# amisr/volumetricinterp

Measured on AMD Instinct MI355X. Metric: fit+eval timesteps/sec, higher is better.
Workload: dtype f64

## Files before the change

### volumetricinterp_amd/csrc/vi_brent.hip

```cpp
#include "vi_solver.h"
#include "vi_jacobi_device.h"
#include "vi_jacobi_v2_device.h"
#include "vi_gemm_device.h"
#include "vi_exp10.h"

#include <cstdlib>
#include <cstring>


#ifdef VI_STAMPS
__device__ unsigned long long g_brent_stamps[16];
__device__ unsigned long long g_brent_hist[64][2];
#define BR_STAMP(k)                                                                   \
    do {                                                                              \
        const unsigned long long t_ = __builtin_readcyclecounter();                   \
        if (threadIdx.x == 0) atomicAdd(&g_brent_stamps[k], t_ - stamp_t);            \
        stamp_t = __builtin_readcyclecounter();                                       \
    } while (0)
#else
#define BR_STAMP(k)
#endif

namespace {

struct BrentState {
    double xpre, xcur, xblk, fpre, fcur, fblk, spre, scur;
    double last_x;
    int it, funcalls, done, status;
    int nreq, rebased, rebase_now;
};

struct RebaseRule {
    double sched[4];
    int nsched;
    int again_after;
    double again_within;
    int again_on;
    double jump_width, jump_frac;
};

__host__ inline int rule_from_host(const double* h, RebaseRule& rr)
{
    rr.nsched = (int)h[0];
    if (rr.nsched < 0 || rr.nsched > 4) return -1;
    for (int i = 0; i < 4; ++i) rr.sched[i] = h[1 + i];
    rr.again_after = (int)h[5];
    rr.again_within = h[6];
    rr.again_on = (int)h[7];
    rr.jump_width = h[8];
    rr.jump_frac = h[9];
    return 0;
}

__host__ __device__ __forceinline__ void rebase_decide(BrentState& s, const RebaseRule& rr)
{
    const double x = s.xcur;
    bool rb = false;
    if (s.last_x == s.last_x) {
        const double d = fabs(x - s.last_x);
        if (s.rebased < rr.nsched)
            rb = d < rr.sched[s.rebased];
        else
            rb = rr.again_on && s.rebased == rr.nsched && s.nreq >= rr.again_after && d < rr.again_within;
    }
// ... 1 lines not shown
    s.rebase_now = rb ? 1 : 0;
    s.last_x = x;
    s.nreq += 1;
}

__host__ __device__ __forceinline__ bool brent_top(BrentState& s, double xtol, double rtol, double jump_width, double jump_fmin)
{
#pragma clang fp contract(off)
    if (s.fpre != 0.0 && s.fcur != 0.0 && (signbit(s.fpre) != signbit(s.fcur))) {
        s.xblk = s.xpre;
        s.fblk = s.fpre;
        s.spre = s.scur = s.xcur - s.xpre;
    }
    if (fabs(s.fblk) < fabs(s.fcur)) {
        const double xp = s.xcur, xc = s.xblk, xb = s.xcur;
        const double fp = s.fcur, fc = s.fblk, fb = s.fcur;
        s.xpre = xp; s.xcur = xc; s.xblk = xb;
        s.fpre = fp; s.fcur = fc; s.fblk = fb;
    }
    const double delta = (xtol + rtol * fabs(s.xcur)) / 2;
    const double sbis = (s.xblk - s.xcur) / 2;
    if (s.fcur == 0.0 || fabs(sbis) < delta) return true;
    if (jump_width > 0.0 && fabs(s.xblk - s.xcur) <= jump_width && fabs(s.fcur) > jump_fmin) return true;
    if (fabs(s.spre) > delta && fabs(s.fcur) < fabs(s.fpre)) {
        double stry;
        if (s.xpre == s.xblk) {
            stry = -s.fcur * (s.xcur - s.xpre) / (s.fcur - s.fpre);
        } else {
            const double dpre = (s.fpre - s.fcur) / (s.xpre - s.xcur);
            const double dblk = (s.fblk - s.fcur) / (s.xblk - s.xcur);
            stry = -s.fcur * (s.fblk * dblk - s.fpre * dpre) / (dblk * dpre * (s.fblk - s.fpre));
        }
        const double a = fabs(s.spre), b = 3 * fabs(sbis) - delta;
        if (2 * fabs(stry) < (b < a ? b : a)) {
            s.spre = s.scur;
            s.scur = stry;
        } else {
            s.spre = sbis;
            s.scur = sbis;
        }
    } else {
        s.spre = sbis;
        s.scur = sbis;
    }
    s.xpre = s.xcur;
    s.fpre = s.fcur;
    if (fabs(s.scur) > delta)
        s.xcur += s.scur;
    else
        s.xcur += (sbis > 0 ? delta : -delta);
    return false;
}

template <int IT>
__device__ __noinline__ void jacobi_system_call(unsigned char* lds_raw, int N, const double* Xs, double sc, const double* ys,
                                                double rcond, double abs_floor, double* Cs, double2* logp, int max_sweeps,
                                                int* sweeps_s, int* nround_s, unsigned long long* round_acc)
{
    if constexpr (IT == 0)
        jacobi_system_v2(lds_raw, N, Xs, sc, ys, rcond, abs_floor, Cs, nullptr, logp, max_sweeps, sweeps_s, nullptr, 0, nround_s,
                         round_acc);
    else
        jacobi_system<IT>(lds_raw, N, Xs, sc, ys, rcond, abs_floor, Cs, nullptr, logp, max_sweeps, sweeps_s, nullptr, 0, nround_s,
                          round_acc);
}

__device__ __noinline__ void rebase_call(unsigned char* lds_raw, int N, const double2* logp, int64_t nround, double* Vs,
                                         double* VwS, double* VnS, const double* AWAr, const double* Rm, double* D1s, double* D2s,
                                         const double* yr, double* yts
#ifdef VI_STAMPS
                                         , unsigned long long& stamp_t
#endif
                                         )
{
    const int tid = threadIdx.x, NT = blockDim.x, nw = NT >> 6, lane = tid & 63, wave = tid >> 6;
    const int NN = N * N;
    for (int col0 = wave * 4; col0 < N; col0 += nw * 4) jacobi_vector_strip<4>(N, logp, nround, col0, lane, VwS);
    __syncthreads();
    BR_STAMP(6);
    double* ldsg = reinterpret_cast<double*>(lds_raw);
    wg_gemm<false>(N, Vs, VwS, VnS, ldsg);
    for (int e = tid; e < NN; e += NT) Vs[e] = VnS[e];
    __syncthreads();
    wg_gemm<false>(N, AWAr, VnS, VwS, ldsg);
    wg_gemm<true>(N, VnS, VwS, D1s, ldsg);
    wg_gemm<false>(N, Rm, VnS, VwS, ldsg);
    wg_gemm<true>(N, VnS, VwS, D2s, ldsg);
    for (int k = wave; k < N; k += nw) {
        double acc = 0.0;
        for (int r = lane; r < N; r += 64) acc = fma(VnS[(int64_t)k * N + r], yr[r], acc);
        for (int o2 = 32; o2 > 0; o2 >>= 1) acc += __shfl_down(acc, o2);
        if (lane == 0) yts[k] = acc;
    }
    __syncthreads();
}

template <int IT>
__global__ __launch_bounds__(IT <= 1 ? 768 : 512) void k_brent_warm(
    int N, int64_t P, int ntask, double* D1, double* D2, double* yt, double* V, const double* __restrict__ AWA,
    const double* __restrict__ Rm, const double* __restrict__ ysrc, RebaseRule rr, double* __restrict__ VwW, double* __restrict__ VnW,
    const double* __restrict__ At, const double* __restrict__ W, const double* __restrict__ b,
    const int* __restrict__ t_rec, const int* __restrict__ t_slot, const double* __restrict__ t_xa,
    const double* __restrict__ t_xb, const double* __restrict__ t_fa, const double* __restrict__ t_fb,
    const double* __restrict__ t_nu, double rcond, double abs_floor, int max_sweeps, double xtol, double rtol, int maxiter,
    int* __restrict__ queue, double* __restrict__ Xw, double2* __restrict__ logw, int64_t log_stride, double* __restrict__ cw,
    double* __restrict__ o_root, double* __restrict__ o_other, int* __restrict__ o_iters, int* __restrict__ o_funcalls,
    int* __restrict__ o_status, size_t lds_jacobi, int npart, unsigned long long* __restrict__ round_acc)
{
    extern __shared__ __align__(16) unsigned char lds_raw[];
    double* shC = reinterpret_cast<double*>(lds_raw + lds_jacobi);
    double* red = shC + ((N + 1) & ~1);
    double* part = red + 768;
    double* shd = part + npart;
    BrentState* st = reinterpret_cast<BrentState*>(shd + 16);
    int* shi = reinterpret_cast<int*>(st + 1);

    const int tid = threadIdx.x, NT = blockDim.x, nw = NT >> 6;
    const int NN = N * N;
    double* Xs = Xw + (int64_t)blockIdx.x * NN;
    double2* logp = logw + (int64_t)blockIdx.x * log_stride;
    double* cp = cw + (int64_t)blockIdx.x * N;
    double* VwS = VwW + (int64_t)blockIdx.x * NN;
    double* VnS = VnW + (int64_t)blockIdx.x * NN;
    const int nb = (int)((P + 255) / 256);

#ifdef VI_STAMPS
    unsigned long long stamp_t = __builtin_readcyclecounter();
    const unsigned long long wall0 = wall_clock64();
    if (threadIdx.x == 0) atomicMin(&g_brent_stamps[12], wall0);
#endif
    for (;;) {
        if (tid == 0) shi[0] = atomicAdd(queue, 1);
        __syncthreads();
        const int task = shi[0];
        if (task >= ntask) {
#ifdef VI_STAMPS
            if (threadIdx.x == 0) { const unsigned long long w1 = wall_clock64(); atomicAdd(&g_brent_stamps[11], w1 - wall0); atomicMax(&g_brent_stamps[13], w1); }
#endif
            break;
        }
        const int64_t slot = t_slot[task], rec = t_rec[task];
        const double nu = t_nu[task];
        double* D1s = D1 + slot * NN;
        double* D2s = D2 + slot * NN;
        double* Vs = V + slot * NN;
        const double* Wr = W + rec * P;
        const double* br = b + rec * P;
        if (tid == 0) {
            BrentState s;
            s.xpre = t_xa[task]; s.xcur = t_xb[task]; s.fpre = t_fa[task]; s.fcur = t_fb[task];
            s.xblk = s.fblk = s.spre = s.scur = 0.0;
            s.it = 1; s.funcalls = 0; s.status = 0;
            s.last_x = __builtin_nan("");
            s.nreq = 0; s.rebased = 0; s.rebase_now = 0;
            s.done = brent_top(s, xtol, rtol, rr.jump_width, rr.jump_frac * nu) ? 1 : 0;
            if (!s.done) rebase_decide(s, rr);
            *st = s;
        }
        __syncthreads();
        BR_STAMP(0);
        while (!st->done) {
            const double alpha = vi_exp10(st->xcur);
            double mx = 0.0;
            for (int e = tid; e < NN; e += NT) mx = fmax(mx, fabs(fma(alpha, D2s[e], D1s[e])));
            for (int o = 32; o > 0; o >>= 1) mx = fmax(mx, __shfl_xor(mx, o));
            if ((tid & 63) == 0) shd[tid >> 6] = mx;
            __syncthreads();
            mx = 0.0;
            for (int q = 0; q < nw; ++q) mx = fmax(mx, shd[q]);
            int ex = 0;
            double f = 1.0;
            if (mx > 0.0 && mx < 1.7e308) {
                (void)frexp(mx, &ex);
                f = ldexp(1.0, 1 - ex);
            }
            for (int e = tid; e < NN; e += NT) Xs[e] = fma(alpha, D2s[e], D1s[e]) * f;
            __syncthreads();
            BR_STAMP(1);
            if constexpr (IT == 3)
                jacobi_system<3>(lds_raw, N, Xs, 1.0 / f, yt + slot * N, rcond, abs_floor, cp, nullptr, logp, max_sweeps, shi + 1,
                                 nullptr, 0, shi + 2, round_acc);
            else
                jacobi_system_call<IT>(lds_raw, N, Xs, 1.0 / f, yt + slot * N, rcond, abs_floor, cp, logp, max_sweeps, shi + 1,
                                       shi + 2, round_acc);
            __syncthreads();
            BR_STAMP(2);
#ifdef VI_STAMPS
            if (tid == 0) { const int ii_ = st->it < 63 ? st->it : 63; atomicAdd(&g_brent_hist[ii_][0], (unsigned long long)shi[1]); atomicAdd(&g_brent_hist[ii_][1], 1ull); atomicAdd(&g_brent_stamps[8], (unsigned long long)shi[1]); atomicAdd(&g_brent_stamps[9], 1ull); atomicAdd(&g_brent_stamps[10], (unsigned long long)shi[2]); }
#endif
            for (int k = tid; k < N; k += NT) red[k] = cp[k];
            __syncthreads();
            for (int r = tid; r < N; r += NT) {
                double acc = 0.0;
                for (int k0 = 0; k0 < N; k0 += 16) {
                    double v[16];
#pragma unroll
                    for (int u = 0; u < 16; ++u) v[u] = (k0 + u < N) ? Vs[(int64_t)(k0 + u) * N + r] : 0.0;
#pragma unroll
                    for (int u = 0; u < 16; ++u)
                        if (k0 + u < N) acc = fma(v[u], red[k0 + u], acc);
                }
                shC[r] = acc;
            }
            __syncthreads();
            BR_STAMP(3);
            const int nbp = NT >> 8;
            for (int b0 = 0; b0 < nb; b0 += nbp) {
                const int sub = tid >> 8, t = tid & 255;
                const int blk = b0 + sub;
                double v = 0.0;
                if (sub < nbp && blk < nb) {
                    const int64_t p = (int64_t)blk * 256 + t;
                    if (p < P) {
                        double acc = 0.0;
#pragma unroll 8
                        for (int n = 0; n < N; ++n) acc = fma(At[(int64_t)n * P + p], shC[n], acc);
                        const double d = acc - br[p];
                        v = d * d * Wr[p];
                    }
                }
                if (sub < nbp) red[tid] = v;
                __syncthreads();
                for (int h = 128; h > 0; h >>= 1) {
                    if (sub < nbp && t < h) red[tid] += red[tid + h];
                    __syncthreads();
                }
                if (sub < nbp && t == 0 && blk < nb) part[blk] = red[tid];
                __syncthreads();
            }
            BR_STAMP(4);
            if (tid == 0) {
                double chi = 0.0;
                for (int j = 0; j < nb; ++j) chi += part[j];
                BrentState s = *st;
                if (shi[1] > max_sweeps) {
                    s.status = 2;
                    s.done = 1;
// ... 195 lines not shown
    h_out[3] = (double)s.funcalls;
    h_out[4] = (double)s.status;
    h_out[5] = (double)s.rebased;
    return VI_OK;
}

extern "C" int vi_brent_warm_f64(vi_ctx* c, int64_t ntask, int32_t N, int64_t P, double* d_D1, double* d_D2, double* d_yt,
                                 double* d_V, const double* d_AWA, const double* d_R, const double* d_y,
                                 const double* h_rebase ,
                                 const double* d_At, const double* d_W,
                                 const double* d_b, const int32_t* d_rec, const int32_t* d_slot, const double* d_xa,
                                 const double* d_xb, const double* d_fa, const double* d_fb, const double* d_nu, double rcond,
                                 double* d_root, double* d_other, int32_t* d_iters, int32_t* d_funcalls, int32_t* d_status)
{
    const double abs_floor = vi_floor_warm();
    const int max_sweeps = vi_max_sweeps();
    size_t ldsj_eff;
    VI_REQUIRE(c && d_D1 && d_D2 && d_yt && d_V && d_AWA && d_R && d_y && h_rebase && d_At && d_W && d_b && d_rec && d_slot && d_xa && d_xb && d_fa && d_fb && d_nu &&
                   d_root && d_other && d_iters && d_funcalls && d_status, "null argument");
    VI_REQUIRE(ntask >= 0 && N > 0 && P > 0, "bad size");
    if (ntask == 0) return VI_OK;
    if (!vi_jacobi_supported(N)) {
        vi_set_error("vi_brent_warm_f64: N=%d outside the in-LDS Jacobi range", N);
        return VI_ERR_UNSUPPORTED;
    }
    int npart;
    const size_t lds_all = brent_lds_bytes(N, P, &ldsj_eff, &npart);
    const size_t shm = lds_all - BRENT_STATIC_LDS;
    if (lds_all > VI_LDS_BYTES_PER_CU) {
        vi_set_error("vi_brent_warm_f64: %lld data points per record need %zu bytes of LDS (the chi^2 partial sums of a record "
                     "sit beside its rotated system); the host-driven iteration has no such limit", (long long)P, lds_all);
        return VI_ERR_UNSUPPORTED;
    }
    VI_HIP(hipSetDevice(c->device));
    int threads, it;
    brent_geometry(N, threads, it);
    const int64_t nwg = ntask < c->n_cu ? ntask : c->n_cu;
    const size_t logb = vi_jacobi_log_bytes(N, max_sweeps);
    double2* logw;
    double *Xw, *VwW, *VnW, *cw;
    int* queue;
    int rc = ws_carve(c, [&](ws_carver& w) {
        logw = w.take<double2>((size_t)nwg * (logb / sizeof(double2)));
        Xw = w.take<double>((size_t)nwg * N * N);
        VwW = w.take<double>((size_t)nwg * N * N);
        VnW = w.take<double>((size_t)nwg * N * N);
        cw = w.take<double>((size_t)nwg * N);
        queue = w.take<int>(1);
    });
    if (rc != VI_OK) return rc;
    RebaseRule rr;
    if (rule_from_host(h_rebase, rr)) { vi_set_error("vi_brent_warm_f64: at most four re-basing thresholds"); return VI_ERR_INVALID; }
    VI_HIP(hipMemsetAsync(queue, 0, sizeof(int), c->stream));
#define VI_B(ITV)                                                                                                             \
    do {                                                                                                                      \
        hipFuncAttributes fattr;                                                                                              \
        VI_HIP(hipFuncGetAttributes(&fattr, (const void*)k_brent_warm<ITV>));                                                 \
        if (fattr.sharedSizeBytes > BRENT_STATIC_LDS) {                                                                       \
            vi_set_error("vi_brent_warm_f64: the kernel has %zu bytes of static LDS, BRENT_STATIC_LDS says %zu",             \
                         (size_t)fattr.sharedSizeBytes, BRENT_STATIC_LDS);                                                    \
            return VI_ERR_UNSUPPORTED;                                                                                        \
        }                                                                                                                     \
        VI_HIP(hipFuncSetAttribute((const void*)k_brent_warm<ITV>, hipFuncAttributeMaxDynamicSharedMemorySize, (int)shm));    \
        hipLaunchKernelGGL(k_brent_warm<ITV>, dim3((unsigned)nwg), dim3(threads), shm, c->stream, N, P, (int)ntask, d_D1, d_D2, \
                           d_yt, d_V, d_AWA, d_R, d_y, rr, VwW, VnW, d_At, d_W, d_b, d_rec, d_slot, d_xa, d_xb, d_fa, d_fb, d_nu, rcond, abs_floor,          \
                           (int)max_sweeps, 2e-12, 4 * 2.220446049250313e-16, 100, queue, Xw, logw,                           \
                           (int64_t)(logb / sizeof(double2)), cw, d_root, d_other, d_iters, d_funcalls, d_status, ldsj_eff, npart, \
                           c->solve_timing ? c->d_rounds : nullptr);                                                        \
    } while (0)
    const int tslot = (int)(c->solve_launches % vi_ctx::NSOLVE_EV);
    if (c->solve_timing) VI_HIP(hipEventRecord(c->evs[tslot][0], c->stream));
    if (it == 0) VI_B(0);
    else if (it <= 1) VI_B(1);
    else if (it <= 2) VI_B(2);
    else VI_B(3);
#undef VI_B
    VI_HIP(hipGetLastError());
    if (c->solve_timing) {
        VI_HIP(hipEventRecord(c->evs[tslot][1], c->stream));
        c->solve_launches += 1;
        c->solve_systems += ntask;
    }
    return VI_OK;
}
```

### volumetricinterp_amd/csrc/vi_jacobi.hip

```cpp
#include "vi_common.h"
#include "vi_solver.h"

#include <cstdlib>
#include <cstring>

#ifdef VI_STAMPS
__device__ unsigned long long g_jacobi_stamps[16];
#define VI_STAMP(k)                                                                          \
    do {                                                                                     \
        const unsigned long long t_ = __builtin_readcyclecounter();                          \
        if (blockIdx.x == 0 && (threadIdx.x == 0 || threadIdx.x == blockDim.x - 64))         \
            g_jacobi_stamps[(threadIdx.x == 0 ? 0 : 8) + (k)] += t_ - stamp_t;               \
        stamp_t = __builtin_readcyclecounter();                                              \
    } while (0)
__device__ unsigned long long g_jacobi_phases[16];
#define VI_PHASE(k)                                                                                          \
    do {                                                                                                     \
        const unsigned long long t_ = __builtin_readcyclecounter();                                          \
        if (threadIdx.x == 0) atomicAdd(&g_jacobi_phases[(conv_tol > 0.0 ? 0 : 8) + (k)], t_ - phase_t);     \
        phase_t = __builtin_readcyclecounter();                                                              \
    } while (0)
#define VI_PHASE_COUNT()                                                                                     \
    do { if (threadIdx.x == 0) atomicAdd(&g_jacobi_phases[(conv_tol > 0.0 ? 0 : 8) + 7], 1ull); } while (0)
#else
#define VI_STAMP(k)
#endif

#ifdef VI_ROTHIST
__device__ unsigned long long g_rot_hist[32][2];
#define VI_ROT_COUNT(sweep, r0, r1, r2, r3)                                                                              \
    atomicAdd(&g_rot_hist[(sweep) < 31 ? (sweep) : 31][0],                                                               \
              (unsigned long long)(((r0).y != 0.0) + ((r1).y != 0.0) + ((r2).y != 0.0) + ((r3).y != 0.0)))
#define VI_ROT_SWEEP(sweep)                                                                                               \
    do { if (threadIdx.x == 0) atomicAdd(&g_rot_hist[(sweep) < 31 ? (sweep) : 31][1], 1ull); } while (0)
#endif

#include "vi_jacobi_device.h"
#include "vi_jacobi_v2_device.h"
#include <cstdlib>
#include <cstring>

namespace {

template <int IT>
__global__ __launch_bounds__(IT == 1 ? 768 : 512) void k_jacobi_solve(
    int N, const double* __restrict__ X, const double* __restrict__ scl, const double* __restrict__ y,
    const int* __restrict__ rec, double rcond, double abs_floor, double* __restrict__ C, int* __restrict__ rank,
    double2* __restrict__ rotlog, int64_t log_stride, int max_sweeps, int* __restrict__ sweeps_out,
    double* __restrict__ lam_out, int lam_raw, int* __restrict__ nround_out, unsigned long long* __restrict__ round_acc,
    double conv_tol)
{
    extern __shared__ __align__(16) unsigned char lds_raw[];
    const int64_t sys = blockIdx.x;
    jacobi_system<IT>(lds_raw, N, X + sys * (int64_t)N * N, scl ? scl[sys] : 1.0, y + (int64_t)(rec ? rec[sys] : sys) * N, rcond,
                      abs_floor, C + sys * N, rank ? rank + sys : nullptr, rotlog + sys * log_stride, max_sweeps,
                      sweeps_out ? sweeps_out + sys : nullptr, lam_out ? lam_out + sys * N : nullptr, lam_raw,
                      nround_out ? nround_out + sys : nullptr, round_acc, conv_tol);
}

__global__ __launch_bounds__(768) void k_jacobi_solve_v2(
    int N, const double* __restrict__ X, const double* __restrict__ scl, const double* __restrict__ y,
    const int* __restrict__ rec, double rcond, double abs_floor, double* __restrict__ C, int* __restrict__ rank,
    double2* __restrict__ rotlog, int64_t log_stride, int max_sweeps, int* __restrict__ sweeps_out,
    double* __restrict__ lam_out, int lam_raw, int* __restrict__ nround_out, unsigned long long* __restrict__ round_acc,
    double conv_tol)
{
    extern __shared__ __align__(16) unsigned char lds_raw[];
    const int64_t sys = blockIdx.x;
    jacobi_system_v2<V2_REPLAY_AHEAD>(lds_raw, N, X + sys * (int64_t)N * N, scl ? scl[sys] : 1.0,
                                      y + (int64_t)(rec ? rec[sys] : sys) * N, rcond, abs_floor, C + sys * N,
                                      rank ? rank + sys : nullptr, rotlog + sys * log_stride, max_sweeps,
                                      sweeps_out ? sweeps_out + sys : nullptr, lam_out ? lam_out + sys * N : nullptr, lam_raw,
                                      nround_out ? nround_out + sys : nullptr, round_acc, conv_tol);
}

template <int CPW>
__global__ __launch_bounds__(64) void k_jacobi_vectors_wave(int N, const double2* __restrict__ rotlog, int64_t log_stride,
                                                            const int* __restrict__ nround_in, double* __restrict__ Vout)
{
    const int64_t sys = blockIdx.y;
    jacobi_vector_strip<CPW>(N, rotlog + sys * log_stride, nround_in[sys], blockIdx.x * CPW, threadIdx.x,
                             Vout + sys * (int64_t)N * N);
}

}

#ifdef VI_STAMPS
extern "C" int vi_debug_jacobi_stamps(double* out, int reset)
{
    unsigned long long h[16];
    if (hipMemcpyFromSymbol(h, HIP_SYMBOL(g_jacobi_stamps), sizeof(h)) != hipSuccess) return -1;
    for (int i = 0; i < 16; ++i) out[i] = (double)h[i];
    if (reset) {
        memset(h, 0, sizeof(h));
        if (hipMemcpyToSymbol(HIP_SYMBOL(g_jacobi_stamps), h, sizeof(h)) != hipSuccess) return -1;
    }
    return 0;
}
#endif

#ifdef VI_STAMPS
extern "C" int vi_debug_jacobi_phases(double* out, int reset)
{
    unsigned long long h[16];
    if (hipMemcpyFromSymbol(h, HIP_SYMBOL(g_jacobi_phases), sizeof(h)) != hipSuccess) return -1;
    for (int i = 0; i < 16; ++i) out[i] = (double)h[i];
    if (reset) {
        memset(h, 0, sizeof(h));
        if (hipMemcpyToSymbol(HIP_SYMBOL(g_jacobi_phases), h, sizeof(h)) != hipSuccess) return -1;
    }
    return 0;
}
#endif

#ifdef VI_ROTHIST
extern "C" int vi_debug_rot_hist(double* out, int reset)
{
    unsigned long long h[32][2];
    if (hipMemcpyFromSymbol(h, HIP_SYMBOL(g_rot_hist), sizeof(h)) != hipSuccess) return -1;
    for (int i = 0; i < 32; ++i) { out[2 * i] = (double)h[i][0]; out[2 * i + 1] = (double)h[i][1]; }
    if (reset) {
        memset(h, 0, sizeof(h));
        if (hipMemcpyToSymbol(HIP_SYMBOL(g_rot_hist), h, sizeof(h)) != hipSuccess) return -1;
    }
    return 0;
}
#endif

namespace {

int jacobi_nsb(int N)
{
    const int M = ((N + 3) & ~3) / 4;
    return M * (M - 1) / 2;
}
void jacobi_geometry(int N, int& threads, int& it)
{
    const int nsb = jacobi_nsb(N);
    if (nsb <= 768) {
        it = 1;
        threads = ((nsb + 63) / 64) * 64;
        if (threads < 64) threads = 64;
    } else {
        threads = 512;
        it = (nsb + 511) / 512;
    }
}

}

bool vi_jacobi_use_v2(int N)
{
    static const bool v1 = vi_env_is("VINTERP_K3", "v1");
    if (v1) return false;
    int threads, it;
    jacobi_geometry(N, threads, it);
    const int M = ((N + 3) & ~3) / 4;
    static const int minm = [] { const int v = vi_env_int("VINTERP_K3_MINM", 24); return v < 3 ? 3 : v; }();
    return it == 1 && M >= minm && M <= 64 && threads + 64 <= 768;
}

size_t vi_jacobi_lds_bytes(int N)
{
    const int Np = (N + 3) & ~3, M = Np / 4;
    const int nt = Np * (Np + 1) / 2;
    size_t b = (size_t)(nt + 2 * Np) * 8 + (size_t)4 * M * 16 + 16 * 8;
    if (vi_jacobi_use_v2(N)) b += (size_t)4 * M * 16 + (size_t)4 * M * 8 + 16 + (size_t)14 * M * 4;
    return (b + 15) & ~(size_t)15;
}

bool vi_jacobi_supported(int N)
{
    int threads, it;
    jacobi_geometry(N, threads, it);
    return N >= 8 && vi_jacobi_lds_bytes(N) <= 159 * 1024 && it <= 3 && ((N + 3) / 4) <= 64;
}

static int64_t jacobi_log_stride(int N, int max_sweeps)
{
    const int Np = (N + 3) & ~3, m = Np / 2, M = Np / 4;
    return (int64_t)max_sweeps * m * 4 * M;
}
size_t vi_jacobi_log_bytes(int N, int max_sweeps) { return (size_t)jacobi_log_stride(N, max_sweeps) * sizeof(double2); }

template <int IT>
static int launch_jacobi(vi_ctx* c, int threads, int64_t B, int N, const double* d_X, const double* d_scl, const double* d_y,
                         const int* d_rec, double rcond, double* d_C, int* d_rank, void* d_log, int max_sweeps,
                         int* d_sweeps, double* d_lam, int lam_raw, int* d_nround, double abs_floor, int64_t log_stride_in,
                         double conv_tol)
{
    const size_t shm = vi_jacobi_lds_bytes(N);
    VI_HIP(hipFuncSetAttribute((const void*)k_jacobi_solve<IT>, hipFuncAttributeMaxDynamicSharedMemorySize, (int)shm));
    const int64_t log_stride = log_stride_in > 0 ? log_stride_in : jacobi_log_stride(N, max_sweeps);
    const int slot = (int)(c->solve_launches % vi_ctx::NSOLVE_EV);
    if (c->solve_timing) VI_HIP(hipEventRecord(c->evs[slot][0], c->stream));
    hipLaunchKernelGGL(k_jacobi_solve<IT>, dim3((unsigned)B), dim3(threads), shm, c->stream, N, d_X, d_scl, d_y, d_rec,
                       rcond, abs_floor, d_C, d_rank, (double2*)d_log, log_stride, max_sweeps, d_sweeps, d_lam, lam_raw, d_nround,
                       c->solve_timing ? c->d_rounds : nullptr, conv_tol);
    VI_HIP(hipGetLastError());
    if (c->solve_timing) {
        VI_HIP(hipEventRecord(c->evs[slot][1], c->stream));
        c->solve_launches += 1;
        c->solve_systems += B;
    }
    return VI_OK;
}

int vi_jacobi_solve(vi_ctx* c, int64_t B, int N, const double* d_X, const double* d_scl, const double* d_y,
                    const int* d_rec, double rcond, double* d_C, int* d_rank, void* d_log, int max_sweeps,
                    int* d_sweeps, double* d_lam, int lam_raw, int* d_nround, double abs_floor, int64_t log_stride, double conv_tol)
{
    int threads, it;
    jacobi_geometry(N, threads, it);
    if (vi_jacobi_use_v2(N)) {
        const size_t shm = vi_jacobi_lds_bytes(N);
        VI_HIP(hipFuncSetAttribute((const void*)k_jacobi_solve_v2, hipFuncAttributeMaxDynamicSharedMemorySize, (int)shm));
        const int64_t ls = log_stride > 0 ? log_stride : jacobi_log_stride(N, max_sweeps);
        const int slot = (int)(c->solve_launches % vi_ctx::NSOLVE_EV);
        if (c->solve_timing) VI_HIP(hipEventRecord(c->evs[slot][0], c->stream));
        hipLaunchKernelGGL(k_jacobi_solve_v2, dim3((unsigned)B), dim3(threads + 64), shm, c->stream, N, d_X, d_scl, d_y, d_rec, rcond,
                           abs_floor, d_C, d_rank, (double2*)d_log, ls, max_sweeps, d_sweeps, d_lam, lam_raw, d_nround,
                           c->solve_timing ? c->d_rounds : nullptr, conv_tol);
        VI_HIP(hipGetLastError());
        if (c->solve_timing) {
            VI_HIP(hipEventRecord(c->evs[slot][1], c->stream));
            c->solve_launches += 1;
            c->solve_systems += B;
        }
        return VI_OK;
    }
#define VI_J(IT) return launch_jacobi<IT>(c, threads, B, N, d_X, d_scl, d_y, d_rec, rcond, d_C, d_rank, d_log, max_sweeps, d_sweeps, d_lam, lam_raw, d_nround, abs_floor, log_stride, conv_tol)
    if (it <= 1) VI_J(1);
    if (it <= 2) VI_J(2);
    VI_J(3);
#undef VI_J
}

bool vi_jacobi_vectors_supported(int N) { return vi_jacobi_supported(N); }

int vi_jacobi_vectors(vi_ctx* c, int64_t B, int N, const void* d_log, int max_sweeps, const int* d_nround, double* d_V,
                      int64_t log_stride_in)
{
    const int64_t log_stride = log_stride_in > 0 ? log_stride_in : jacobi_log_stride(N, max_sweeps);
    const int64_t cols = B * N, target = (int64_t)8 * c->n_cu;
#define VI_VEC(CPW)                                                                                                           \
    hipLaunchKernelGGL(k_jacobi_vectors_wave<CPW>, dim3((unsigned)((N + CPW - 1) / CPW), (unsigned)B), dim3(64), 0, c->stream, \
                       N, (const double2*)d_log, log_stride, d_nround, d_V)
    if (cols <= target) VI_VEC(1);
    else if (cols <= 2 * target) VI_VEC(2);
    else if (cols <= 4 * target) VI_VEC(4);
    else VI_VEC(8);
#undef VI_VEC
    VI_HIP(hipGetLastError());
    return VI_OK;
}
```

### volumetricinterp_amd/csrc/vi_jacobi_v2_device.h

```cpp
#pragma once
#include "vi_jacobi_device.h"

namespace {

__device__ __forceinline__ void lds_signal(int* w, int n)
{
    asm volatile("s_waitcnt lgkmcnt(0)" ::: "memory");
    __hip_atomic_fetch_add(w, n, __ATOMIC_RELAXED, __HIP_MEMORY_SCOPE_WORKGROUP);
}
template <bool SLEEP = true>
__device__ __forceinline__ void lds_wait(int* w, int target, int& bad)
{
    const int tgt = __builtin_amdgcn_readfirstlane(target);
    int spins = 0;
#pragma nounroll
    for (;;) {
        const int v = __builtin_amdgcn_readfirstlane(__hip_atomic_load(w, __ATOMIC_RELAXED, __HIP_MEMORY_SCOPE_WORKGROUP));
        if (v >= tgt) break;
        if (++spins > (1 << 22)) { bad = 1; break; }
        if (SLEEP) __builtin_amdgcn_s_sleep(1);
    }
    asm volatile("" ::: "memory");
}


struct V2Frame {
    int N, NT, Np, m, M, nsb, ntri, dg, tid, nw;
    double* A;
    double* yv;
    double2* cs0;
    double* nd;
    double* mb;
    int* sync;
    int* dtab;
    __device__ __forceinline__ V2Frame(unsigned char* lds_raw, int N_)
    {
        N = N_;
        NT = blockDim.x;
        Np = (N + 3) & ~3;
        m = Np >> 1;
        M = Np >> 2;
        nsb = (M * (M - 1)) >> 1;
        ntri = 16 * nsb + 10 * M;
        dg = 16 * nsb;
        A = reinterpret_cast<double*>(lds_raw);
        yv = A + ntri;
        cs0 = reinterpret_cast<double2*>(yv + 2 * Np);
        nd = reinterpret_cast<double*>(cs0 + 8 * M);
        mb = nd + 16;
        sync = reinterpret_cast<int*>(mb + 4 * M);
        dtab = sync + 4;
        tid = threadIdx.x;
        nw = NT >> 6;
    }
// ... 432 lines not shown
#pragma unroll
                    for (int j = 0; j < 4; ++j) pf[u][j] = lp[j * M];
                }
            }
#pragma unroll
            for (int u = 0; u < PF; ++u)
                if (u < nb) W.round(pf[u], ((r1 - 1 - u) % m) == 0);
        }
    }
    return W;
}

template <int DEPTH>
__device__ __forceinline__ WaveReplay v2_replay_ahead(const V2Frame& f, const V2Run& run, const double2* __restrict__ logp)
{
    const int m = f.m, M = f.M, tid = f.tid;
    const int nround = (int)run.nround;
    const double* yc = f.yv + run.ycur * f.Np;
    WaveReplay W;
    W.init(tid, M);
    W.load(yc, M);
    const bool has = tid < M;
    const double2* lbase = logp + (has ? tid : 0);
    double2 pf[DEPTH][4];
    auto issue = [&](double2 (&p)[4], int rr) {
        const double2* lp = lbase + (rr > 0 ? rr : 0) * (int64_t)(4 * M);
#pragma unroll
        for (int j = 0; j < 4; ++j) p[j] = lp[j * M];
    };
    int rm = nround > 0 ? (nround - 1) % m : 0;
    auto apply = [&](const double2 (&p)[4]) {
        double2 q[4];
#pragma unroll
        for (int j = 0; j < 4; ++j) q[j] = has ? p[j] : make_double2(1.0, 0.0);
        W.round(q, rm == 0);
        rm = rm == 0 ? m - 1 : rm - 1;
    };
#pragma unroll
    for (int u = 0; u < DEPTH; ++u) issue(pf[u], nround - 1 - u);
    int r1 = nround;
    for (; r1 >= DEPTH; r1 -= DEPTH) {
#pragma unroll
        for (int u = 0; u < DEPTH; ++u) {
            apply(pf[u]);
            issue(pf[u], r1 - 1 - u - DEPTH);
        }
    }
#pragma unroll
    for (int u = 0; u < DEPTH; ++u)
        if (u < r1) apply(pf[u]);
    return W;
}

#ifndef VI_PHASE
#define VI_PHASE(k)
#define VI_PHASE_COUNT()
#endif

template <int AHEAD = 0>
__device__ __forceinline__ void jacobi_system_v2(
    unsigned char* lds_raw, int N, const double* __restrict__ Xs, double sc, const double* __restrict__ ys, double rcond,
    double abs_floor, double* __restrict__ Cs, int* __restrict__ rank_s, double2* __restrict__ logp, int max_sweeps,
    int* __restrict__ sweeps_s, double* __restrict__ lam_s, int lam_raw, int* __restrict__ nround_s,
    unsigned long long* __restrict__ round_acc, double conv_tol = 0.0)
{
    const V2Frame f(lds_raw, N);
    V2Geo g;
#ifdef VI_STAMPS
    unsigned long long phase_t = __builtin_readcyclecounter();
#endif
    v2_setup(f, g);
    VI_PHASE(0);
    const double mxd = v2_load_close(f, v2_load_rows(f, Xs, ys, f.yv, f.tid >> 6, f.nw, f.tid, f.NT));
    VI_PHASE(1);
    const double drop = rcond * mxd;
    const double eps2 = 2.220446049250313e-16 * 2.220446049250313e-16;
    const double conv2 = conv_tol > 0.0 ? conv_tol * conv_tol : VI_CONV_FACTOR * VI_CONV_FACTOR * eps2;
    V2Run run;
    run.ycur = 0;
    v2_iterate(f, g, drop, abs_floor, conv2, max_sweeps, logp, run);
    VI_PHASE(2);
    v2_truncate(f, run, sc, rcond, rank_s, max_sweeps, sweeps_s, lam_s, lam_raw, nround_s, round_acc);
    VI_PHASE(3);
    double* yc = f.yv + run.ycur * f.Np;
    if (f.tid < 64) {
        if (AHEAD > 0) v2_replay_ahead<(AHEAD > 0 ? AHEAD : 1)>(f, run, logp).store(yc, f.M);
        else v2_replay(f, run, logp).store(yc, f.M);
    }
    VI_PHASE(4);
    __syncthreads();
    for (int s = f.tid; s < N; s += f.NT) Cs[s] = yc[s];
    VI_PHASE(5);
    VI_PHASE_COUNT();
}

constexpr int V2_REPLAY_AHEAD = 8;

}
```

### volumetricinterp_amd/csrc/vi_solver.h

```cpp
#pragma once
#include "vi_common.h"

size_t vi_jacobi_lds_bytes(int N);
size_t vi_jacobi_log_bytes(int N, int max_sweeps);
bool vi_jacobi_supported(int N);
bool vi_jacobi_use_v2(int N);
int vi_jacobi_solve(vi_ctx* c, int64_t B, int N, const double* d_X, const double* d_scl, const double* d_y,
                    const int* d_rec, double rcond, double* d_C, int* d_rank, void* d_log, int max_sweeps,
                    int* d_sweeps, double* d_lam, int lam_raw, int* d_nround, double abs_floor, int64_t log_stride = 0,
                    double conv_tol = 0.0);
bool vi_jacobi_vectors_supported(int N);
int vi_jacobi_vectors(vi_ctx* c, int64_t B, int N, const void* d_log, int max_sweeps, const int* d_nround, double* d_V,
                      int64_t log_stride = 0);

bool vi_qr_supported(int N);
size_t vi_qr_hh_bytes(int N);
int vi_qr_precond(vi_ctx* c, int64_t B, int N, const double* d_X, const double* d_y, const int* d_rec, double* d_X1,
                  double* d_y1, double* d_hh, double* d_scr, int64_t hh_stride = 0);
int vi_qr_back_vec(vi_ctx* c, int64_t B, int N, const double* d_hh, double* d_C, int64_t hh_stride = 0);
int vi_qr_back_mat(vi_ctx* c, int64_t B, int N, const double* d_hh, double* d_V, int64_t hh_stride = 0);

int vi_walk_rotate(vi_ctx* c, int64_t B, int N, const double* d_AWA, const int* d_rec, const double* d_V, const double* d_D2,
                   const int* d_basis, const double* d_y, const double* d_alpha, double* d_X, double* d_scl, double* d_yt);

double vi_floor_warm();

int vi_eval_sph_mfma(vi_model* m, int64_t Q, const double* lat, const double* lon, const double* alt, int64_t T,
                     const double* Cp, const unsigned char* hull, int F, double* out, int64_t* done);
int vi_eval_sph_split(vi_model* m, int64_t Q, const double* lat, const double* lon, const double* alt, int64_t T,
                      const double* Cp, const unsigned char* hull, int F, double* out, int* handled);
int vi_eval_resident_mfma(vi_ctx* c, int N, int64_t Q, int64_t T, const double* d_Y, const double* d_C, double* d_out, int* handled);
int vi_eval_resident_err_mfma(vi_ctx* c, int N, int64_t Q, int64_t T, const double* d_Y, const double* d_dC, double* d_out,
                              int* handled);
int vi_eval_resident_err_at_mfma(vi_ctx* c, int N, int64_t outer, int64_t L, int64_t inner, int64_t T, const double* d_Y,
                                 const double* d_dC, const int32_t* d_idx, double* d_out, int* handled);
bool vi_eval_records_err_shape(int N, int64_t Q, const double* d_Y, const double* d_out);
int vi_eval_records_err_mfma(vi_ctx* c, int N, int64_t Q, const double* d_Y, const int32_t* d_rec, const double* d_w, int64_t R,
                             const double* d_dC, double* d_out, int* handled);
bool vi_eval_resident_gradcov_shape(int N);
int vi_eval_resident_gradcov_mfma(vi_ctx* c, int N, int64_t Q, int64_t T, const double* d_G, const double* d_dC, double* d_out,
                                  int64_t ldo, int* handled);
int vi_eval_records_gradcov_mfma(vi_ctx* c, int N, int64_t Q, const double* d_G, const int32_t* d_rec, const double* d_w, int64_t R,
                                 const double* d_dC, double* d_out, int64_t ldo, int* handled);
bool vi_peak_fused_shape(int N, int64_t outer, int64_t L, int64_t inner);
size_t vi_peak_fused_work_bytes(int64_t outer, int64_t L, int64_t T);
int vi_eval_resident_peak_mfma(vi_ctx* c, int N, int64_t outer, int64_t L, int64_t T, const double* d_Y, const double* d_C, int kind,
                               double* d_val, int32_t* d_idx, void* d_work, size_t work_bytes, int* handled);
int vi_peak_columns(vi_ctx* c, int64_t outer, int64_t L, int64_t inner, int64_t T, int kind, const double* d_in, double* d_val,
                    int32_t* d_idx);
int vi_reduce_basis(vi_ctx* c, int N, int64_t outer, int64_t L, int64_t inner, const double* d_Y, const double* d_w, double* d_Yr);

#define VI_INTERNAL __attribute__((visibility("hidden")))
VI_INTERNAL int prepare_call(vi_model* m, int64_t Q, const double* d_lat, const double* d_lon, const double* d_alt,
                             const double* d_hull_eq, int32_t F, double hull_tol, int64_t rows, const double* d_C);
VI_INTERNAL int grad_model_check(const vi_model* m, const char* who);
VI_INTERNAL int launch_grad_resident(vi_model* m, const char* who, int64_t Q, const double* d_lat, const double* d_lon,
                                     const double* d_alt, const unsigned char* d_mask, int32_t frame, double* d_G);
VI_INTERNAL int mask_basis(vi_model* m, int64_t Q, const unsigned char* d_mask, double* d_Y);
struct GradcovChunks { int64_t chunk; double *G, *work; };
// ... 19 lines not shown
```

Baseline: 3643.

## Add staged producer-consumer LDS ring for Jacobi rotation replay in Brent kernel

Adds a staged replay mode for the Jacobi v2 rotation replay. The otherwise idle waves act as producers that prefetch rotation-log entries from global memory into an LDS ring buffer, while wave 0 consumes them and applies the rotations. This is meant to hide global-memory latency in the serial replay phase that a single wave previously did alone. The Brent warm kernel defaults to this staged mode, and the standalone solve keeps the ahead mode. The cost is added LDS signalling and spin-wait synchronisation, plus a fallback flag if waits fail.

```diff
diff --git a/volumetricinterp_amd/csrc/vi_brent.hip b/volumetricinterp_amd/csrc/vi_brent.hip
--- a/volumetricinterp_amd/csrc/vi_brent.hip
+++ b/volumetricinterp_amd/csrc/vi_brent.hip
@@ -1,4 +1,14 @@
 #include "vi_solver.h"
+#ifdef VI_STAMPS
+__device__ unsigned long long g_brent_stamps[16];
+#define VI_PHASE(k)                                                                             \
+    do {                                                                                        \
+        const unsigned long long t_ = __builtin_readcyclecounter();                             \
+        if (((k) == 4 || (k) == 2) && threadIdx.x == 0) atomicAdd(&g_brent_stamps[(k) == 4 ? 14 : 15], t_ - phase_t); \
+        phase_t = __builtin_readcyclecounter();                                                 \
+    } while (0)
+#define VI_PHASE_COUNT()
+#endif
 #include "vi_jacobi_device.h"
 #include "vi_jacobi_v2_device.h"
 #include "vi_gemm_device.h"
@@ -9,7 +19,6 @@
 
 
 #ifdef VI_STAMPS
-__device__ unsigned long long g_brent_stamps[16];
 __device__ unsigned long long g_brent_hist[64][2];
 #define BR_STAMP(k)                                                                   \
     do {                                                                              \
@@ -117,14 +126,14 @@
     return false;
 }
 
-template <int IT>
+template <int IT, int REPLAY>
 __device__ __noinline__ void jacobi_system_call(unsigned char* lds_raw, int N, const double* Xs, double sc, const double* ys,
                                                 double rcond, double abs_floor, double* Cs, double2* logp, int max_sweeps,
-                                                int* sweeps_s, int* nround_s, unsigned long long* round_acc)
+                                                int* sweeps_s, int* nround_s, unsigned long long* round_acc, int ring_cap)
 {
     if constexpr (IT == 0)
-        jacobi_system_v2(lds_raw, N, Xs, sc, ys, rcond, abs_floor, Cs, nullptr, logp, max_sweeps, sweeps_s, nullptr, 0, nround_s,
-                         round_acc);
+        jacobi_system_v2<REPLAY>(lds_raw, N, Xs, sc, ys, rcond, abs_floor, Cs, nullptr, logp, max_sweeps, sweeps_s, nullptr, 0,
+                                 nround_s, round_acc, 0.0, ring_cap);
     else
         jacobi_system<IT>(lds_raw, N, Xs, sc, ys, rcond, abs_floor, Cs, nullptr, logp, max_sweeps, sweeps_s, nullptr, 0, nround_s,
                           round_acc);
@@ -160,7 +169,7 @@
     __syncthreads();
 }
 
-template <int IT>
+template <int IT, int REPLAY = V2_REPLAY_PLAIN>
 __global__ __launch_bounds__(IT <= 1 ? 768 : 512) void k_brent_warm(
     int N, int64_t P, int ntask, double* D1, double* D2, double* yt, double* V, const double* __restrict__ AWA,
     const double* __restrict__ Rm, const double* __restrict__ ysrc, RebaseRule rr, double* __restrict__ VwW, double* __restrict__ VnW,
@@ -170,7 +179,7 @@
     const double* __restrict__ t_nu, double rcond, double abs_floor, int max_sweeps, double xtol, double rtol, int maxiter,
     int* __restrict__ queue, double* __restrict__ Xw, double2* __restrict__ logw, int64_t log_stride, double* __restrict__ cw,
     double* __restrict__ o_root, double* __restrict__ o_other, int* __restrict__ o_iters, int* __restrict__ o_funcalls,
-    int* __restrict__ o_status, size_t lds_jacobi, int npart, unsigned long long* __restrict__ round_acc)
+    int* __restrict__ o_status, size_t lds_jacobi, int npart, unsigned long long* __restrict__ round_acc, int ring_cap)
 {
     extern __shared__ __align__(16) unsigned char lds_raw[];
     double* shC = reinterpret_cast<double*>(lds_raw + lds_jacobi);
@@ -246,8 +255,8 @@
                 jacobi_system<3>(lds_raw, N, Xs, 1.0 / f, yt + slot * N, rcond, abs_floor, cp, nullptr, logp, max_sweeps, shi + 1,
                                  nullptr, 0, shi + 2, round_acc);
             else
-                jacobi_system_call<IT>(lds_raw, N, Xs, 1.0 / f, yt + slot * N, rcond, abs_floor, cp, logp, max_sweeps, shi + 1,
-                                       shi + 2, round_acc);
+                jacobi_system_call<IT, REPLAY>(lds_raw, N, Xs, 1.0 / f, yt + slot * N, rcond, abs_floor, cp, logp, max_sweeps,
+                                               shi + 1, shi + 2, round_acc, ring_cap);
             __syncthreads();
             BR_STAMP(2);
 #ifdef VI_STAMPS
@@ -549,26 +558,31 @@
     RebaseRule rr;
     if (rule_from_host(h_rebase, rr)) { vi_set_error("vi_brent_warm_f64: at most four re-basing thresholds"); return VI_ERR_INVALID; }
     VI_HIP(hipMemsetAsync(queue, 0, sizeof(int), c->stream));
-#define VI_B(ITV)                                                                                                             \
+#define VI_B(...)                                                                                                             \
     do {                                                                                                                      \
         hipFuncAttributes fattr;                                                                                              \
-        VI_HIP(hipFuncGetAttributes(&fattr, (const void*)k_brent_warm<ITV>));                                                 \
+        auto kern_ = k_brent_warm<__VA_ARGS__>;                                                                               \
+        VI_HIP(hipFuncGetAttributes(&fattr, (const void*)kern_));                                                             \
         if (fattr.sharedSizeBytes > BRENT_STATIC_LDS) {                                                                       \
             vi_set_error("vi_brent_warm_f64: the kernel has %zu bytes of static LDS, BRENT_STATIC_LDS says %zu",             \
                          (size_t)fattr.sharedSizeBytes, BRENT_STATIC_LDS);                                                    \
             return VI_ERR_UNSUPPORTED;                                                                                        \
         }                                                                                                                     \
-        VI_HIP(hipFuncSetAttribute((const void*)k_brent_warm<ITV>, hipFuncAttributeMaxDynamicSharedMemorySize, (int)shm));    \
-        hipLaunchKernelGGL(k_brent_warm<ITV>, dim3((unsigned)nwg), dim3(threads), shm, c->stream, N, P, (int)ntask, d_D1, d_D2, \
+        VI_HIP(hipFuncSetAttribute((const void*)kern_, hipFuncAttributeMaxDynamicSharedMemorySize, (int)shm));                \
+        hipLaunchKernelGGL(kern_, dim3((unsigned)nwg), dim3(threads), shm, c->stream, N, P, (int)ntask, d_D1, d_D2,           \
                            d_yt, d_V, d_AWA, d_R, d_y, rr, VwW, VnW, d_At, d_W, d_b, d_rec, d_slot, d_xa, d_xb, d_fa, d_fb, d_nu, rcond, abs_floor,          \
                            (int)max_sweeps, 2e-12, 4 * 2.220446049250313e-16, 100, queue, Xw, logw,                           \
                            (int64_t)(logb / sizeof(double2)), cw, d_root, d_other, d_iters, d_funcalls, d_status, ldsj_eff, npart, \
-                           c->solve_timing ? c->d_rounds : nullptr);                                                        \
+                           c->solve_timing ? c->d_rounds : nullptr, vi_k3_ring_cap());                                      \
     } while (0)
     const int tslot = (int)(c->solve_launches % vi_ctx::NSOLVE_EV);
     if (c->solve_timing) VI_HIP(hipEventRecord(c->evs[tslot][0], c->stream));
-    if (it == 0) VI_B(0);
-    else if (it <= 1) VI_B(1);
+    if (it == 0) {
+        const int replay = vi_k3_replay_mode(true);
+        if (replay == V2_REPLAY_STAGED) VI_B(0, V2_REPLAY_STAGED);
+        else if (replay == V2_REPLAY_AHEAD) VI_B(0, V2_REPLAY_AHEAD);
+        else VI_B(0, V2_REPLAY_PLAIN);
+    } else if (it <= 1) VI_B(1);
     else if (it <= 2) VI_B(2);
     else VI_B(3);
 #undef VI_B
diff --git a/volumetricinterp_amd/csrc/vi_jacobi.hip b/volumetricinterp_amd/csrc/vi_jacobi.hip
--- a/volumetricinterp_amd/csrc/vi_jacobi.hip
+++ b/volumetricinterp_amd/csrc/vi_jacobi.hip
@@ -58,20 +58,20 @@
                       nround_out ? nround_out + sys : nullptr, round_acc, conv_tol);
 }
 
+template <int REPLAY>
 __global__ __launch_bounds__(768) void k_jacobi_solve_v2(
     int N, const double* __restrict__ X, const double* __restrict__ scl, const double* __restrict__ y,
     const int* __restrict__ rec, double rcond, double abs_floor, double* __restrict__ C, int* __restrict__ rank,
     double2* __restrict__ rotlog, int64_t log_stride, int max_sweeps, int* __restrict__ sweeps_out,
     double* __restrict__ lam_out, int lam_raw, int* __restrict__ nround_out, unsigned long long* __restrict__ round_acc,
-    double conv_tol)
+    double conv_tol, int ring_cap)
 {
     extern __shared__ __align__(16) unsigned char lds_raw[];
     const int64_t sys = blockIdx.x;
-    jacobi_system_v2<V2_REPLAY_AHEAD>(lds_raw, N, X + sys * (int64_t)N * N, scl ? scl[sys] : 1.0,
-                                      y + (int64_t)(rec ? rec[sys] : sys) * N, rcond, abs_floor, C + sys * N,
-                                      rank ? rank + sys : nullptr, rotlog + sys * log_stride, max_sweeps,
-                                      sweeps_out ? sweeps_out + sys : nullptr, lam_out ? lam_out + sys * N : nullptr, lam_raw,
-                                      nround_out ? nround_out + sys : nullptr, round_acc, conv_tol);
+    jacobi_system_v2<REPLAY>(lds_raw, N, X + sys * (int64_t)N * N, scl ? scl[sys] : 1.0, y + (int64_t)(rec ? rec[sys] : sys) * N,
+                             rcond, abs_floor, C + sys * N, rank ? rank + sys : nullptr, rotlog + sys * log_stride, max_sweeps,
+                             sweeps_out ? sweeps_out + sys : nullptr, lam_out ? lam_out + sys * N : nullptr, lam_raw,
+                             nround_out ? nround_out + sys : nullptr, round_acc, conv_tol, ring_cap);
 }
 
 template <int CPW>
@@ -158,6 +158,42 @@
     const int M = ((N + 3) & ~3) / 4;
     static const int minm = [] { const int v = vi_env_int("VINTERP_K3_MINM", 24); return v < 3 ? 3 : v; }();
     return it == 1 && M >= minm && M <= 64 && threads + 64 <= 768;
+}
+
+constexpr int K3_REPLAY_DEFAULT_SOLVE = V2_REPLAY_AHEAD, K3_REPLAY_DEFAULT_BRENT = V2_REPLAY_STAGED;
+int vi_k3_replay_mode(bool brent)
+{
+    static const int forced = vi_env_is("VINTERP_K3_REPLAY", "plain") ? 0 : vi_env_is("VINTERP_K3_REPLAY", "ahead") ? 1
+                              : vi_env_is("VINTERP_K3_REPLAY", "staged") ? 2 : -1;
+    if (forced >= 0) return forced;
+    return brent ? K3_REPLAY_DEFAULT_BRENT : K3_REPLAY_DEFAULT_SOLVE;
+}
+int vi_k3_ring_cap()
+{
+    static const int v = [] { const int s = vi_env_int("VINTERP_K3_RING", 0); return s < 0 ? 0 : s; }();
+    return v;
+}
+
+extern "C" int vi_k3_ring_plan(int32_t N, int32_t threads, int32_t ring_cap, int32_t nround, int32_t* hdr, int32_t* plan)
+{
+    if (N < 9 || nround < 0 || !hdr || (nround > 0 && !plan)) return VI_ERR_INVALID;
+    const int Np = (N + 3) & ~3, M = Np / 4, ntri = Np * (Np + 1) / 2;
+    int th, it;
+    jacobi_geometry(N, th, it);
+    const int nw = (threads > 0 ? threads : th + 64) / 64;
+    const int slots = k3_ring_slots(ntri, M, ring_cap), nprod = nw - 1;
+    hdr[0] = slots;
+    hdr[1] = nprod;
+    hdr[2] = k3_ring_usable(slots, nprod, M) ? 1 : 0;
+    if (!hdr[2]) return VI_OK;
+    for (int i = 0; i < nround; ++i) {
+        plan[5 * i] = k3_ring_round(nround, i);
+        plan[5 * i + 1] = k3_ring_slot(i, slots);
+        plan[5 * i + 2] = k3_ring_producer(i, nprod);
+        plan[5 * i + 3] = k3_ring_filled_target(i, nprod);
+        plan[5 * i + 4] = k3_ring_free_target(i, slots);
+    }
+    return VI_OK;
 }
 
 size_t vi_jacobi_lds_bytes(int N)
@@ -214,13 +250,16 @@
     jacobi_geometry(N, threads, it);
     if (vi_jacobi_use_v2(N)) {
         const size_t shm = vi_jacobi_lds_bytes(N);
-        VI_HIP(hipFuncSetAttribute((const void*)k_jacobi_solve_v2, hipFuncAttributeMaxDynamicSharedMemorySize, (int)shm));
+        const int replay = vi_k3_replay_mode(false);
+        auto kern = replay == V2_REPLAY_STAGED ? k_jacobi_solve_v2<V2_REPLAY_STAGED>
+                    : replay == V2_REPLAY_AHEAD ? k_jacobi_solve_v2<V2_REPLAY_AHEAD> : k_jacobi_solve_v2<V2_REPLAY_PLAIN>;
+        VI_HIP(hipFuncSetAttribute((const void*)kern, hipFuncAttributeMaxDynamicSharedMemorySize, (int)shm));
         const int64_t ls = log_stride > 0 ? log_stride : jacobi_log_stride(N, max_sweeps);
         const int slot = (int)(c->solve_launches % vi_ctx::NSOLVE_EV);
         if (c->solve_timing) VI_HIP(hipEventRecord(c->evs[slot][0], c->stream));
-        hipLaunchKernelGGL(k_jacobi_solve_v2, dim3((unsigned)B), dim3(threads + 64), shm, c->stream, N, d_X, d_scl, d_y, d_rec, rcond,
+        hipLaunchKernelGGL(kern, dim3((unsigned)B), dim3(threads + 64), shm, c->stream, N, d_X, d_scl, d_y, d_rec, rcond,
                            abs_floor, d_C, d_rank, (double2*)d_log, ls, max_sweeps, d_sweeps, d_lam, lam_raw, d_nround,
-                           c->solve_timing ? c->d_rounds : nullptr, conv_tol);
+                           c->solve_timing ? c->d_rounds : nullptr, conv_tol, vi_k3_ring_cap());
         VI_HIP(hipGetLastError());
         if (c->solve_timing) {
             VI_HIP(hipEventRecord(c->evs[slot][1], c->stream));
diff --git a/volumetricinterp_amd/csrc/vi_jacobi_v2_device.h b/volumetricinterp_amd/csrc/vi_jacobi_v2_device.h
--- a/volumetricinterp_amd/csrc/vi_jacobi_v2_device.h
+++ b/volumetricinterp_amd/csrc/vi_jacobi_v2_device.h
@@ -1,5 +1,6 @@
 #pragma once
 #include "vi_jacobi_device.h"
+#include "vi_k3_ring.h"
 
 namespace {
 
@@ -538,17 +539,113 @@
     return W;
 }
 
+template <int PD>
+__device__ __forceinline__ void v2_replay_staged(const V2Frame& f, const V2Run& run, const double2* __restrict__ logp, int slots,
+                                                 double* yc, int& bad)
+{
+    constexpr int KMAX = 3;
+    const int m = f.m, M = f.M, tid = f.tid, per = 4 * f.M;
+    const int nround = (int)run.nround, nprod = f.nw - 1;
+    double2* ring = reinterpret_cast<double2*>(f.A);
+    int* cnt = reinterpret_cast<int*>(f.mb);
+    if (tid < 64) {
+        WaveReplay W;
+        W.init(tid, M);
+        W.load(yc, M);
+        const bool has = tid < M;
+        const double2* rb = ring + (has ? tid : 0);
+        int rm = nround > 0 ? (nround - 1) % m : 0;
+        double2 qn[4];
+        auto fetch = [&](int slot) __attribute__((always_inline)) {
+            const double2* sp = rb + slot * per;
+#pragma unroll
+            for (int j = 0; j < 4; ++j) qn[j] = sp[j * M];
+        };
+        int p1 = 0, t1 = 1, s1 = 0;
+        auto advance = [&]() __attribute__((always_inline)) {
+            if (++p1 == nprod) { p1 = 0; ++t1; }
+            if (++s1 == slots) s1 = 0;
+        };
+        if (nround > 0) {
+            lds_wait<false>(cnt + 1 + p1, t1, bad);
+            fetch(s1);
+            advance();
+        }
+#pragma nounroll
+        for (int i = 0; i < nround && !bad; ++i) {
+            double2 q[4];
+#pragma unroll
+            for (int j = 0; j < 4; ++j) q[j] = has ? qn[j] : make_double2(1.0, 0.0);
+            if (tid == 0) lds_signal(cnt, 1);
+            if (i + 1 < nround) {
+                lds_wait<false>(cnt + 1 + p1, t1, bad);
+                fetch(s1);
+                advance();
+            }
+            W.round(q, rm == 0);
+            rm = rm == 0 ? m - 1 : rm - 1;
+        }
+        W.store(yc, M);
+    } else {
+        const int lane = tid & 63, pw = (tid >> 6) - 1;
+        static_assert(PD == 4, "four named buffers");
+        typedef double v2d __attribute__((ext_vector_type(2)));
+        struct Buf { v2d a, b, c; } v0, v1, v2, v3;
+        static_assert(KMAX == 3, "Buf holds three entries");
+        const int o0 = lane, o1 = lane + 64 < per ? lane + 64 : 0, o2 = lane + 128 < per ? lane + 128 : 0;
+        auto issue = [&](Buf& p, int i) __attribute__((always_inline)) {
+            const int r = k3_ring_round(nround, i);
+            typedef const v2d __attribute__((address_space(1)))* glog;
+            const glog src = (glog)(logp + (r > 0 ? r : 0) * (int64_t)per);
+            p.a = src[o0];
+            p.b = src[o1];
+            p.c = src[o2];
+        };
+        issue(v0, pw);
+        issue(v1, pw + nprod);
+        issue(v2, pw + 2 * nprod);
+        issue(v3, pw + 3 * nprod);
+        int i = pw, slot = pw % slots;
+        const int sstep = nprod % slots;
+        auto stage = [&](Buf& p) __attribute__((always_inline)) {
+            if (i < nround && !bad) {
+                if (i >= slots) lds_wait(cnt, k3_ring_free_target(i, slots), bad);
+                v2d* dp = reinterpret_cast<v2d*>(ring + slot * per);
+                if (lane < per) dp[lane] = p.a;
+                if (lane + 64 < per) dp[lane + 64] = p.b;
+                if (lane + 128 < per) dp[lane + 128] = p.c;
+                if (lane == 0) lds_signal(cnt + 1 + pw, 1);
+                issue(p, i + PD * nprod);
+            }
+            i += nprod;
+            slot += sstep;
+            if (slot >= slots) slot -= slots;
+        };
+#pragma nounroll
+        while (i < nround && !bad) {
+            stage(v0);
+            stage(v1);
+            stage(v2);
+            stage(v3);
+        }
+    }
+}
+
 #ifndef VI_PHASE
 #define VI_PHASE(k)
 #define VI_PHASE_COUNT()
 #endif
 
-template <int AHEAD = 0>
+enum { V2_REPLAY_PLAIN = 0, V2_REPLAY_AHEAD = 1, V2_REPLAY_STAGED = 2 };
+constexpr int V2_AHEAD_DEPTH = 8;
+constexpr int V2_STAGED_DEPTH = 4;
+
+template <int REPLAY = V2_REPLAY_PLAIN>
 __device__ __forceinline__ void jacobi_system_v2(
     unsigned char* lds_raw, int N, const double* __restrict__ Xs, double sc, const double* __restrict__ ys, double rcond,
     double abs_floor, double* __restrict__ Cs, int* __restrict__ rank_s, double2* __restrict__ logp, int max_sweeps,
     int* __restrict__ sweeps_s, double* __restrict__ lam_s, int lam_raw, int* __restrict__ nround_s,
-    unsigned long long* __restrict__ round_acc, double conv_tol = 0.0)
+    unsigned long long* __restrict__ round_acc, double conv_tol = 0.0, int ring_cap = 0)
 {
     const V2Frame f(lds_raw, N);
     V2Geo g;
@@ -566,20 +663,28 @@
     run.ycur = 0;
     v2_iterate(f, g, drop, abs_floor, conv2, max_sweeps, logp, run);
     VI_PHASE(2);
+    const int slots = k3_ring_slots(f.ntri, f.M, ring_cap);
+    const bool staged = REPLAY == V2_REPLAY_STAGED && k3_ring_usable(slots, f.nw - 1, f.M);
+    if (staged && f.tid < 16) reinterpret_cast<int*>(f.mb)[f.tid] = 0;
     v2_truncate(f, run, sc, rcond, rank_s, max_sweeps, sweeps_s, lam_s, lam_raw, nround_s, round_acc);
     VI_PHASE(3);
     double* yc = f.yv + run.ycur * f.Np;
-    if (f.tid < 64) {
-        if (AHEAD > 0) v2_replay_ahead<(AHEAD > 0 ? AHEAD : 1)>(f, run, logp).store(yc, f.M);
-        else v2_replay(f, run, logp).store(yc, f.M);
-    }
-    VI_PHASE(4);
-    __syncthreads();
+    if (staged) {
+        int bad = 0;
+        v2_replay_staged<V2_STAGED_DEPTH>(f, run, logp, slots, yc, bad);
+        VI_PHASE(4);
+        if (__syncthreads_or(bad) && f.tid == 0 && sweeps_s) *sweeps_s = max_sweeps + 1;
+    } else {
+        if (f.tid < 64) {
+            if (REPLAY == V2_REPLAY_AHEAD) v2_replay_ahead<V2_AHEAD_DEPTH>(f, run, logp).store(yc, f.M);
+            else v2_replay(f, run, logp).store(yc, f.M);
+        }
+        VI_PHASE(4);
+        __syncthreads();
+    }
     for (int s = f.tid; s < N; s += f.NT) Cs[s] = yc[s];
     VI_PHASE(5);
     VI_PHASE_COUNT();
 }
 
-constexpr int V2_REPLAY_AHEAD = 8;
-
-}
+}
diff --git a/volumetricinterp_amd/csrc/vi_k3_ring.h b/volumetricinterp_amd/csrc/vi_k3_ring.h
--- /dev/null
+++ b/volumetricinterp_amd/csrc/vi_k3_ring.h
@@ -0,0 +1,20 @@
+#pragma once
+
+#if defined(__HIPCC__) || defined(__CUDACC__)
+#define VI_RING_HD __host__ __device__ __forceinline__
+#else
+#define VI_RING_HD inline
+#endif
+
+VI_RING_HD int k3_ring_slots(int ntri, int M, int cap)
+{
+    int s = ntri / (8 * M);
+    if (cap > 0 && s > cap) s = cap;
+    return s;
+}
+VI_RING_HD int k3_ring_round(int nround, int i) { return nround - 1 - i; }
+VI_RING_HD int k3_ring_slot(int i, int slots) { return i % slots; }
+VI_RING_HD int k3_ring_producer(int i, int nprod) { return i % nprod; }
+VI_RING_HD int k3_ring_filled_target(int i, int nprod) { return i / nprod + 1; }
+VI_RING_HD int k3_ring_free_target(int i, int slots) { return i - slots + 1; }
+VI_RING_HD bool k3_ring_usable(int slots, int nprod, int M) { return slots >= 2 && nprod >= 1 && 4 * M <= 192; }
diff --git a/volumetricinterp_amd/csrc/vi_solver.h b/volumetricinterp_amd/csrc/vi_solver.h
--- a/volumetricinterp_amd/csrc/vi_solver.h
+++ b/volumetricinterp_amd/csrc/vi_solver.h
@@ -5,6 +5,8 @@
 size_t vi_jacobi_log_bytes(int N, int max_sweeps);
 bool vi_jacobi_supported(int N);
 bool vi_jacobi_use_v2(int N);
+int vi_k3_replay_mode(bool brent);
+int vi_k3_ring_cap();
 int vi_jacobi_solve(vi_ctx* c, int64_t B, int N, const double* d_X, const double* d_scl, const double* d_y,
                     const int* d_rec, double rcond, double* d_C, int* d_rank, void* d_log, int max_sweeps,
                     int* d_sweeps, double* d_lam, int lam_raw, int* d_nround, double abs_floor, int64_t log_stride = 0,
```

Result: faster. 3686 (median of 6 runs) (+1.2%).
